# HKUST-KnowComp/DualMessagePassing

Hardware: AMD Instinct MI355X
Metric: (pattern,graph) pairs/sec DMPNN fwd+bwd hid=128 (higher is better)
Workload: dtype f32

## Files before the change

### dualmessagepassing_amd/_abi.py

```python
import ctypes

c_int = ctypes.c_int
c_i32 = ctypes.c_int32
c_i64 = ctypes.c_int64
c_u64 = ctypes.c_uint64
c_f32 = ctypes.c_float
c_double = ctypes.c_double
c_ptr = ctypes.c_void_p
c_size = ctypes.c_size_t

ABI_VERSION = 90

DMP_COLLATE_MAX_JOBS = 4
DMP_POOL_MAX_JOBS = 4
DMP_REDUCE_MAX_SEGMENTS = 16
DMP_ADAMW_MAX_SKIP = 16
DMP_ADAMW_MAX_SEGMENTS = 1024
DMP_LOOKUP_MAX_JOBS = 8
DMP_CONCAT_MAX_JOBS = 12
DMP_GEMM_MAX_JOBS = 12
DMP_GEMM_MAX_TERMS = 3
DMP_ATB_MAX_JOBS = 8
DMP_MEM_MEAN, DMP_MEM_SUM, DMP_MEM_MAX = 0, 1, 2


class dmp_collate_job(ctypes.Structure):
    _fields_ = [("local_src", c_ptr), ("local_dst", c_ptr), ("num_nodes", c_ptr), ("num_edges", c_ptr), ("B", c_i64), ("N", c_i64),
                ("E", c_i64), ("node_off", c_ptr), ("edge_off", c_ptr), ("src", c_ptr), ("dst", c_ptr), ("edge_graph", c_ptr),
                ("node_graph", c_ptr)]


class dmp_pool_job(ctypes.Structure):
    _fields_ = [("sizes_a", c_ptr), ("sizes_b", c_ptr), ("Ba", c_i64), ("Bb", c_i64), ("flag_a", c_ptr), ("flag_b", c_ptr),
                ("rows_a", c_i64), ("R", c_i64), ("chunk", c_int), ("off", c_ptr), ("gptr", c_ptr), ("vptr", c_ptr), ("vent", c_ptr),
                ("gent", c_ptr), ("seg", c_ptr), ("flag8", c_ptr), ("rowmap", c_ptr), ("sizes", c_ptr)]


class dmp_smallk_job(ctypes.Structure):
    _fields_ = [("X", c_ptr), ("ldx", c_i64), ("D", c_ptr), ("ldd", c_i64), ("gate", c_ptr), ("rowmask", c_ptr), ("R", c_i64),
                ("partial", c_ptr)]


class dmp_l0_pack_job(ctypes.Structure):
    _fields_ = [("enc_p", c_ptr), ("ldp", c_i64), ("rows_p", c_i64), ("enc_g", c_ptr), ("ldg", c_i64), ("gate", c_ptr), ("rows_g", c_i64),
# ... 233 lines not shown
    "dmp_atb_typed_blocks_h": (c_i64, [c_i64, c_int]),
    "dmp_atb_rows_blocks_h": (c_i64, [c_i64, c_int, c_int, c_int]),
    "dmp_atb_rows_plain": (c_int, [c_ptr, c_i64, c_ptr, c_i64, c_ptr, c_i64, c_int, c_int, c_int, c_ptr, c_ptr]),
    "dmp_atb_rows_masked": (c_int, [c_ptr, c_i64, c_ptr, c_i64, c_ptr, c_ptr, c_i64, c_int, c_int, c_int, c_ptr, c_ptr, c_ptr]),
    "dmp_atb_jobs_blocks_h": (c_i64, [c_i64, c_int, c_int]),
    "dmp_atb_rows_jobs_h": (c_int, [_p(dmp_atb_job), c_int, c_i64, c_int, c_ptr, c_ptr, c_ptr, c_i64, c_ptr]),
    "dmp_atb_tile_jobs_blocks": (c_i64, [c_i64, c_int, c_int]),
    "dmp_mfma_partial_rows_h": (c_i64, [c_i64, c_int]),
    "dmp_gemm_k64": (c_int, [c_ptr, c_i64, c_ptr, c_i64, c_int, c_ptr, c_i64, c_i64, c_ptr]),
    "dmp_atb_typed": (c_int, [c_ptr, c_i64, c_ptr, c_i64, c_ptr, c_ptr, c_ptr, c_i64, c_i64, c_int, c_ptr, c_ptr, c_ptr]),
    "dmp_out_fwd_fused_rows": (c_int, [c_ptr, c_i64, c_ptr, c_i64, c_ptr, c_ptr, c_ptr, c_int, c_ptr, c_i64, c_i64, c_int, c_int, c_ptr,
                                       c_i64, c_ptr]),
    "dmp_bwd_h1_fused_rows": (c_int, [c_ptr, c_i64, c_ptr, c_i64, c_ptr, c_i64, c_ptr, c_ptr, c_ptr, c_int, c_i64, c_int, c_f32, c_ptr,
                                      c_i64, c_ptr, c_ptr, c_ptr]),
    "dmp_kept_rows_scratch_words": (c_i64, [c_i64]),
    "dmp_kept_rows": (c_int, [c_ptr, c_i64, c_int, c_ptr, c_ptr, c_ptr, c_ptr]),
    "dmp_l0_edge_fwd_rows": (c_int, [c_ptr, c_i64, c_int, c_ptr, c_i64, c_ptr, c_i64, c_ptr, c_ptr, c_ptr, c_ptr, c_ptr, c_ptr, c_i64, c_int,
                                     c_f32, c_ptr, c_i64, c_ptr]),
    "dmp_l0_bwd_w_rows": (c_int, [c_ptr, c_i64, c_int, c_ptr, c_ptr, c_i64, c_ptr, c_i64, c_ptr, c_ptr, c_i64, c_int, c_ptr, c_ptr]),
    "dmp_typed_partial_rows": (c_i64, [c_i64, c_int]),
    "dmp_out_fwd_typed": (c_int, [_p(dmp_typed_job), c_int, c_ptr, c_ptr, c_ptr, c_i64, c_i64, c_int, c_ptr]),
    "dmp_bwd_h1_typed": (c_int, [c_ptr, c_i64, c_ptr, c_i64, c_ptr, c_i64, c_ptr, c_ptr, c_ptr, c_i64, c_i64, c_int, c_f32, c_ptr, c_i64,
                                 c_ptr, c_ptr, c_ptr]),
    "dmp_kept_rows_jobs": (c_int, [_p(dmp_kept_job), c_int, c_ptr, c_ptr, c_ptr, c_ptr, c_i64, c_ptr, c_ptr, c_ptr, c_ptr]),
    "dmp_row_mask_bits_jobs": (c_int, [_p(dmp_rowmask_job), c_int, c_ptr]),
    "dmp_atb2_blocks": (c_i64, [c_i64, c_int]),
    "dmp_atb2_jobs": (c_int, [_p(dmp_atb2_job), c_int, c_ptr, c_ptr, c_ptr, c_i64, c_i64, c_int, c_ptr]),
    "dmp_bwd_z_w": (c_int, [c_ptr, c_i64, c_ptr, c_i64, c_ptr, c_i64, c_ptr, c_i64, c_i64, c_ptr, c_i64, c_ptr, c_ptr, c_f32, c_f32,
                            c_ptr, c_ptr, c_ptr, c_i64, c_i64, c_int, c_ptr, c_i64, c_ptr, c_i64, c_ptr, c_ptr]),
    "dmp_out_fwd_typed_codes": (c_int, [_p(dmp_typed_job), c_ptr, c_i64, c_int, c_ptr, c_i64, c_i64, c_i64, c_ptr, c_ptr, c_ptr, c_i64, c_i64, c_int, c_ptr]),
    "dmp_bwd_h1_w_blocks": (c_i64, [c_i64]),
    "dmp_bwd_h1_w": (c_int, [c_ptr, c_i64, c_ptr, c_i64, c_ptr, c_i64, c_ptr, c_ptr, c_i64, c_i64, c_int, c_f32, c_ptr, c_i64,
                             c_ptr, c_ptr, c_ptr, c_ptr]),
    "dmp_row_mask_bits": (c_int, [c_ptr, c_i64, c_ptr, c_ptr]),
    "dmp_row_mask_rows": (c_int, [c_ptr, c_i64, c_int, c_i64, c_ptr, c_ptr]),
    "dmp_bwd_z_fused": (c_int, [c_ptr, c_i64, c_ptr, c_i64, c_ptr, c_i64, c_i64, c_ptr, c_i64, c_ptr, c_ptr, c_ptr,
                                c_f32, c_f32, c_i64, c_int, c_ptr, c_i64, c_ptr]),
    "dmp_gemm_k128": (c_int, [c_ptr, c_i64, c_ptr, c_i64, c_int, c_ptr, c_i64, c_i64, c_int, c_ptr]),
    "dmp_edge_combine": (c_int, [c_ptr, c_i64, c_ptr, c_i64, c_ptr, c_ptr, c_ptr, c_ptr, c_ptr, c_i64,
                                 c_int, c_int, c_f32, c_ptr, c_i64, c_ptr]),
    "dmp_relu_bwd_g_colsum": (c_int, [c_ptr, c_i64, c_ptr, c_i64, c_ptr, c_ptr, c_i64, c_int, c_f32, c_ptr, c_i64,
                                      c_ptr, c_ptr]),
    "dmp_edge_combine_bwd_g": (c_int, [c_ptr, c_i64, c_ptr, c_ptr, c_i64, c_int, c_ptr, c_i64, c_ptr]),
    "dmp_compgcn_agg": (c_int, [c_ptr, c_i64, c_ptr, c_i64, c_ptr, c_ptr, c_ptr, c_ptr, c_i64, c_int, c_int,
                                c_ptr, c_i64, c_ptr]),
    "dmp_compgcn_agg_bwd": (c_int, [c_ptr, c_i64, c_ptr, c_i64, c_ptr, c_i64, c_ptr, c_ptr, c_ptr, c_ptr,
                                    c_i64, c_int, c_int, c_ptr, c_i64, c_ptr, c_i64, c_ptr]),
    "dmp_attn_supported_dh": (c_int, [c_int]),
    "dmp_attn_fwd": (c_int, [c_ptr, c_ptr, c_ptr, c_ptr, c_ptr, c_i64, c_i64, c_i64, c_int, c_int, c_f32, c_ptr, c_ptr, c_ptr, c_ptr]),
    "dmp_attn_bwd": (c_int, [c_ptr, c_ptr, c_ptr, c_ptr, c_ptr, c_ptr, c_ptr, c_ptr, c_i64, c_i64, c_i64, c_int, c_int, c_f32, c_ptr,
                             c_ptr, c_ptr, c_ptr, c_ptr]),
    "dmp_mem_init_fwd": (c_int, [c_ptr, c_i64, c_ptr, c_i64, c_ptr, c_i64, c_i64, c_int, c_int, c_int, c_int, c_int, c_ptr, c_ptr,
                                 c_ptr, c_ptr, c_ptr, c_ptr, c_ptr]),
    "dmp_mem_init_bwd": (c_int, [c_ptr, c_ptr, c_ptr, c_ptr, c_ptr, c_i64, c_i64, c_int, c_int, c_int, c_int, c_ptr, c_ptr, c_ptr]),
    "dmp_cnn_fwd": (c_int, [c_ptr, c_i64, c_i64, c_int, c_ptr, c_ptr, c_int, c_int, c_int, c_int, c_int, c_f32, c_ptr, c_int, c_ptr,
                            c_ptr, c_ptr, c_ptr, c_ptr]),
    "dmp_cnn_route_bwd": (c_int, [c_ptr, c_ptr, c_ptr, c_i64, c_i64, c_i64, c_int, c_int, c_int, c_f32, c_ptr, c_ptr]),
    "dmp_cnn_wgrad_chunks": (c_i64, [c_i64]),
    "dmp_cnn_wgrad": (c_int, [c_ptr, c_ptr, c_i64, c_i64, c_i64, c_int, c_int, c_int, c_ptr, c_ptr]),
    "dmp_rnn_fwd": (c_int, [c_ptr, c_ptr, c_ptr, c_ptr, c_ptr, c_i64, c_i64, c_int, c_int, c_int, c_ptr, c_ptr, c_ptr, c_ptr]),
    "dmp_rnn_bwd": (c_int, [c_ptr, c_ptr, c_ptr, c_ptr, c_ptr, c_i64, c_i64, c_int, c_int, c_int, c_ptr, c_ptr]),
    "dmp_relconv_supported": (c_int, [c_int, c_int]),
    "dmp_relconv_fwd": (c_int, [c_ptr, c_ptr, c_ptr, c_ptr, c_ptr, c_ptr, c_ptr, c_i64, c_int, c_int, c_int, c_int, c_int, c_ptr,
                                c_ptr]),
    "dmp_relconv_bwd": (c_int, [c_ptr, c_ptr, c_ptr, c_ptr, c_ptr, c_ptr, c_ptr, c_i64, c_int, c_int, c_int, c_int, c_int, c_ptr,
                                c_ptr]),
# ... 2 lines not shown
```

### dualmessagepassing_amd/_build.py

```python
import fcntl
import hashlib
import os
import shutil
import subprocess
import tempfile

_HERE = os.path.dirname(os.path.abspath(__file__))
CSRC = os.path.join(_HERE, "csrc")
LIB_PATH = os.path.join(CSRC, "libdmp_hip.so")
HASH_PATH = LIB_PATH + ".srchash"
SOURCES = ["dmp_agg.hip", "dmp_segacc.hip", "dmp_compact.hip", "dmp_graph.hip", "dmp_fused.hip", "dmp_mfma.hip", "dmp_typed.hip", "dmp_h1w.hip", "dmp_atb.hip", "dmp_fold.hip", "dmp_heads.hip", "dmp_layer0.hip", "dmp_bn.hip", "dmp_attn.hip", "dmp_mem.hip", "dmp_cnn.hip", "dmp_rnn.hip", "dmp_relconv.hip",
           "dmp_subiso.cpp"]
HEADERS = ["dmp_common.h", "dmp_mfma_common.h", os.path.join("..", "..", "include", "dmp_hip.h")]
ARCH = "gfx950"
FLAGS = ["-O3", "-std=c++17", "-fPIC", "-ffp-contract=off", "-Wall", "-Wno-unused-function"]


def find_hipcc():
    for cand in (os.environ.get("HIPCC"), shutil.which("hipcc"), "/opt/rocm/bin/hipcc"):
        if cand and os.path.exists(cand):
            return cand
    return None


def source_hash():
    h = hashlib.sha256()
    h.update((ARCH + " ".join(FLAGS)).encode())
    for f in SOURCES + HEADERS:
        with open(os.path.join(CSRC, f), "rb") as fh:
            h.update(f.encode())
            h.update(fh.read())
    return h.hexdigest()


def _stale():
    if not os.path.exists(LIB_PATH) or not os.path.exists(HASH_PATH):
        return True
    with open(HASH_PATH) as f:
        return f.read().strip() != source_hash()


def build_lib(force=False, verbose=False):
    if not force and not _stale():
        return LIB_PATH
# ... 43 lines not shown
```

### dualmessagepassing_amd/fused.py

```python
import threading

import torch
from torch.autograd.function import once_differentiable

from . import _abi, _lib, ops
from ._lib import check, ptr, stream_ptr


def _partials(rows, H, dev):
    lib = _lib.load()
    return torch.empty((int(lib.dmp_colsum_partial_rows(rows, H)), H), dtype=torch.float32, device=dev)


MAX_REDUCE_SEGMENTS = _abi.DMP_REDUCE_MAX_SEGMENTS


class _Deferred(threading.local):

    def __init__(self):
        self.stack = []


_deferred = _Deferred()

# ... 617 lines not shown
USE_OUT_CODES = True


def out_codes_ok(h1, enc, K, Wc):
    lib = _lib.load()
    lim = (1 << 32) - 65536
    return bool(USE_OUT_CODES and h1.size(1) == 128 and not lib.dmp_dev_get_exact_fp32() and 1 <= K <= 16 and Wc.size(0) == K and Wc.size(1) == 128
                and enc.dtype == torch.float32 and enc.stride(1) == 1 and enc.stride(0) % 4 == 0 and enc.data_ptr() % 16 == 0
                and enc.size(0) == h1.size(0) and h1.size(0) * 128 * 4 < lim and Wc.stride(1) == 1)


def out_fwd_typed_codes(h1, W2t, b2, enc, K, Wc, tiles, prev=None, out=None, w_in_out=True, row0=0):
    lib = _lib.load()
    slot_edge, tile_scale, num_tiles, bound = tiles
    R, H = h1.shape
    if out is None:
        out = dead_rows_buffer((R, H), h1.device)
    Wc = Wc.detach()
    _lib.require_gpu(h1, W2t, out, prev, b2, enc, Wc)
    j = _abi.dmp_typed_job()
    j.Hin, j.ldh, j.W2, j.ldw, j.w_in_out = h1.data_ptr(), h1.stride(0), W2t.data_ptr(), W2t.stride(0), int(bool(w_in_out))
    j.bias = ptr(b2)
    j.R, j.ldr = ptr(prev), (prev.stride(0) if prev is not None else H)
    j.R2, j.ldr2 = None, H
    j.act, j.slope = 0, 0.0
    j.out, j.ldo = out.data_ptr(), out.stride(0)
    with _lib.timed("out_fwd_typed_codes[H=%d,R=%d]", (H, R), 4 * H * R * 2 + 4 * enc.size(1) * R):
        check(lib.dmp_out_fwd_typed_codes(_ctypes.byref(j), ptr(enc), enc.stride(0), int(K), ptr(Wc), Wc.stride(0), int(row0),
                                          0 if prev is None else min(R, prev.size(0)), ptr(slot_edge), ptr(tile_scale),
                                          ptr(num_tiles), bound, R, H, stream_ptr()), "dmp_out_fwd_typed_codes")
    return out


def out_fwd_typed(h1, W2t, b2, prev, tiles, out=None, w_in_out=True, slope=None, prev2=None):
    R, H = h1.shape
    if out is None:
        out = dead_rows_buffer((R, H), h1.device)
    typed_jobs([dict(a=h1, W=W2t, bias=b2, prev=prev, prev2=prev2, out=out, w_in_out=w_in_out, slope=slope)], tiles)
    return out


def bwd_h1_typed(d_o, W2, h1, tiles, slope=0.0, out=None):
    lib = _lib.load()
    E, H = d_o.shape
    slot_edge, tile_scale, num_tiles, bound = tiles
    d_g = out if out is not None else dead_rows_buffer((E, H), d_o.device)
    G = int(lib.dmp_typed_partial_rows(bound, H))
    part = torch.empty((G, H), dtype=torch.float32, device=d_o.device)
    part_rows = torch.empty_like(part)
    W2 = W2.contiguous()
    with _lib.timed("bwd_h1_typed[H=%d,E=%d]", (H, E), 12 * H * E + 4 * E):
        check(lib.dmp_bwd_h1_typed(ptr(d_o), d_o.stride(0), ptr(W2), W2.size(1), ptr(h1), h1.stride(0), ptr(slot_edge), ptr(tile_scale),
                                   ptr(num_tiles), bound, E, H, slope, ptr(d_g), d_g.stride(0), ptr(part), ptr(part_rows), stream_ptr()),
              "dmp_bwd_h1_typed")
    return d_g, reduce_partials(part), reduce_partials(part_rows)


def h1w_ok(d_o, h1, H):
    lib = _lib.load()
    return (H == 128 and not lib.dmp_dev_get_exact_fp32() and d_o.size(0) * d_o.stride(0) * 4 < (1 << 32) - 65536
            and h1.size(0) * h1.stride(0) * 4 < (1 << 32) - 65536 and d_o.size(0) * H * 4 < (1 << 32) - 65536)


def bwd_h1_w(d_o, W2, h1, tiles, slope=0.0, out=None):
    lib = _lib.load()
    E, H = d_o.shape
    slot_edge, _, num_tiles, bound = tiles
    d_g = out if out is not None else dead_rows_buffer((E, H), d_o.device)
    G = int(lib.dmp_bwd_h1_w_blocks(bound))
    part = torch.empty((G, H), dtype=torch.float32, device=d_o.device)
# ... 787 lines not shown
            XP = torch.empty((N, 3 * H), dtype=torch.float32, device=z.device)
            for t, (n0, n1) in l0.vtables(N):
                smallk_embed(l0.venc[n0:n1, :VK], MV[t * VK:(t + 1) * VK], None, XP[n0:n1], H)
        else:
            XP = x @ Wx
        if l0 is not None and node_pass:
            PXr, ldpx = PX, 2 * H
        else:
            PXr, ldpx = XP[:, H:], 3 * H
            if l0 is not None or nd is None:
                H1n = add_bias_relu_(SB, XP[:, :H], bn, slope)
        if nd is not None:
            xn = dead_rows_buffer((N, H), z.device) if (inner & 1) else torch.zeros((N, H), dtype=torch.float32, device=z.device)
            if nW2t is not None:
                out_fwd_typed(H1n, nW2t, nb2, x if residual else None, nd.tiles, out=xn)
            else:
                out_fwd_typed(H1n, nW2, nb2, x if residual else None, nd.tiles, out=xn, w_in_out=False)
        elif onepanel_ok(H):
            xn = out_fwd_mfma(H1n, nW2, nb2, v_gate, x if residual else None, nW2t)
        else:
            xn = gate_residual(x if residual else None, torch.addmm(nb2, H1n, nW2.t()), v_gate)
        sums_only = epool is not None and not edge_rows
        zn = None
        side.wait("erows" if l0 is not None else "tiles")
        dead_gate = e_gate if (SKIP_DEAD_ROWS and USE_ROW_MASKS and e_gate is not None and typed_ok(index, H)
                               and gate_row_mask(e_gate) is not None) else None
        if l0 is not None:
            H1e = dead_rows_buffer((z.size(0), H), z.device) if dead_gate is not None else torch.empty((z.size(0), H), dtype=torch.float32, device=z.device)
            for t, rows, _ in tables:
                if rows[1] > rows[0]:
                    l0_edge_fwd(enc0, K0, M0[t * K0:(t + 1) * K0], PXr, ldpx, be, coef, index, slope, rows, H1e,
                                mask=gate_row_mask(dead_gate) if dead_gate is not None else None)
        elif typed_ok(index, H):
            H1e = edge_fwd_typed(z, Wes, PXr, ldpx, be, coef, index, slope, dead_gate=dead_gate, sel=None if nd is None else nd.sel)
        elif mfma_ok(index, H):
            H1e = edge_fwd_mfma(z, Wes, PXr, ldpx, be, coef, index, slope)
        else:
            G = z @ Wes
            H1e = edge_combine_raw(G, 2 * H, PXr, ldpx, be, coef, index, H, relu=True, slope=slope)
            del G
            if not sums_only:
                Oe = torch.addmm(eb2, H1e, eW2.t())
                zn = gate_residual(z if residual else None, Oe, e_gate)
        if zn is None and not sums_only:
            dead = (3 if (inner & 1) else 1) if (dead_gate is not None and zero_rows_gate(e_gate)) else 0
            side.wait("tiles")
            lt = live_tiles(index, coef, e_gate) if (dead == 3 and eW2t is not None) else None
            if lt is not None:
                tl_ = ascending_tiles(e_gate) or lt
                if l0 is not None and residual and getattr(l0, "z_from_codes", False) and out_codes_ok(H1e, l0.enc, l0.K, W0[-l0.K:]):
                    zn = out_fwd_typed_codes(H1e, eW2t, eb2, l0.enc, l0.K, W0[-l0.K:], tl_, prev=l0.z_head, row0=l0.z_head.size(0))
                else:
                    zn = out_fwd_typed(H1e, eW2t, eb2, l0_rows(l0, W0, z) if residual else None, tl_)
            elif (l0 is not None and residual and e_gate is None and getattr(l0, "z_from_codes", False) and eW2t is not None
                  and out_codes_ok(H1e, l0.enc, l0.K, W0[-l0.K:]) and identity_tiles(H1e.size(0), H1e.device) is not None):
                zn = out_fwd_typed_codes(H1e, eW2t, eb2, l0.enc, l0.K, W0[-l0.K:], identity_tiles(H1e.size(0), H1e.device), prev=l0.z_head,
                                         row0=l0.z_head.size(0))
            else:
                zn = out_fwd_mfma(H1e, eW2, eb2, e_gate, l0_rows(l0, W0, z) if residual else None, eW2t, dead_rows=dead)
        ctx.index, ctx.coef, ctx.residual, ctx.H = index, coef, residual, H
        ctx.v_gate, ctx.e_gate, ctx.WesT, ctx.slope = v_gate, e_gate, WesT, slope
        ctx.vpool, ctx.epool = vpool, epool
        ctx.inner = int(inner)
        ctx.nd = nd
        ctx.l0, ctx.l0_S0, ctx.l0_tables = l0, S0, tables
        ctx.l0_W = None if l0 is None else (W0.detach(), None if WV0 is None else WV0.detach())
        ctx.save_for_backward(x, z if l0 is None else None, S, H1n, H1e, Bn, Wx, Wes, nW2, eW2)
# ... 315 lines not shown
```

### include/dmp_hip.h

```cpp
#ifndef DMP_HIP_H
#define DMP_HIP_H

#include <stddef.h>
#include <stdint.h>

#ifdef __cplusplus
extern "C" {
#endif

#define DMP_OK 0
#define DMP_ERR_BAD_ARG (-1)
#define DMP_ERR_UNSUPPORTED (-2)
#define DMP_ERR_HIP (-3)

#define DMP_ABI_VERSION 90
int dmp_abi_version(void);
const char *dmp_last_hip_error(void);


size_t dmp_csr_workspace_words(int64_t num_nodes, int64_t num_edges);

int dmp_csr_build(const int64_t *key, const uint8_t *flag, int64_t num_edges,
                  int64_t num_nodes, int32_t *rowptr, int32_t *ent,
                  int32_t *key32, int64_t *degree, int32_t *status,
                  int32_t *ws, void *stream);

size_t dmp_csr_pair_workspace_words(int64_t num_nodes);
int dmp_csr_build_pair(const int64_t *dst, const int64_t *src, const uint8_t *flag, int64_t num_edges, int64_t num_nodes,
                       int32_t *in_ptr, int32_t *in_ent, int32_t *dst32, int64_t *in_deg,
                       int32_t *out_ptr, int32_t *out_ent, int32_t *src32, int64_t *out_deg,
                       int32_t *status, int32_t *ws, void *stream);

int dmp_csr_build_graphs_max_nodes(void);
int dmp_csr_build_graphs(const int64_t *dst, const int64_t *src, const uint8_t *flag, const int64_t *node_off,
                         const int64_t *edge_off, int64_t B, int64_t E, int64_t N, int32_t *in_ptr, int32_t *in_ent,
                         int32_t *dst32, int64_t *in_deg, int32_t *out_ptr, int32_t *out_ent, int32_t *src32,
                         int64_t *out_deg, int32_t *status, void *stream);

int dmp_incidence_build(const int32_t *in_ptr, const int32_t *in_ent,
                        const int32_t *out_ptr, const int32_t *out_ent,
                        int64_t num_nodes, int64_t num_edges, int32_t *inc_ptr,
                        int32_t *inc_ent, void *stream);

int dmp_degree_coef(const int64_t *out_deg, int64_t num_nodes, float *coef,
                    void *stream);

int dmp_collate(const int64_t *local_src, const int64_t *local_dst,
                const int64_t *num_nodes, const int64_t *num_edges,
// ... 433 lines not shown
  const float *bias;
  const float *R; int64_t ldr;
  const float *R2; int64_t ldr2;
  int act; float slope;
  float *out; int64_t ldo;
} dmp_typed_job;
int dmp_out_fwd_typed(const dmp_typed_job *jobs, int num_jobs, const int32_t *slot_edge, const float *tile_scale,
                      const int32_t *num_tiles, int64_t tiles_bound, int64_t E, int H, void *stream);
int dmp_bwd_h1_typed(const float *dO, int64_t ldo, const float *W2, int64_t ldw, const float *H1, int64_t ldh,
                     const int32_t *slot_edge, const float *tile_scale, const int32_t *num_tiles, int64_t tiles_bound, int64_t E,
                     int H, float slope, float *dG, int64_t ldg, float *partial, float *partial_rows, void *stream);
int dmp_out_fwd_typed_codes(const dmp_typed_job *job, const float *codes, int64_t ldc, int kcodes, const float *Wc, int64_t ldwc,
                            int64_t code_row0, int64_t r_rows, const int32_t *slot_edge, const float *tile_scale, const int32_t *num_tiles, int64_t tiles_bound, int64_t E,
                            int H, void *stream);

typedef struct {
  const float *Z; int64_t ldz;
  const float *D; int64_t ldd;
  float *partial_T, *partial_B; int64_t partial_stride; int ldp;
} dmp_atb2_job;
int64_t dmp_atb2_blocks(int64_t tiles_bound, int num_jobs);
int dmp_atb2_jobs(const dmp_atb2_job *jobs, int num_jobs, const int32_t *slot_row, const float *tile_scale, const int32_t *num_tiles,
                  int64_t tiles_bound, int64_t rows, int H, void *stream);

int dmp_bwd_z_w(const float *dPre, int64_t ldp, const float *Z, int64_t ldz, const float *W, int64_t ldw, const float *D, int64_t ldd,
                int64_t num_nodes, const float *base, int64_t ldb, const int32_t *dst, const uint8_t *flag, float s0, float s1,
                const int32_t *slot_edge, const float *tile_scale, const int32_t *num_tiles, int64_t tiles_bound, int64_t E, int H,
                const int32_t *base_map, int64_t base_rows, float *dZ, int64_t ldo, float *partial_w, void *stream);
int64_t dmp_bwd_h1_w_blocks(int64_t tiles_bound);
int dmp_bwd_h1_w(const float *dO, int64_t ldo, const float *W2, int64_t ldw, const float *H1, int64_t ldh,
                 const int32_t *slot_edge, const int32_t *num_tiles, int64_t tiles_bound, int64_t E, int H, float slope,
                 float *dG, int64_t ldg, float *partial, float *partial_rows, float *partial_w, void *stream);

int dmp_bwd_z_fused(const float *dPre, int64_t ldp, const float *W, int64_t ldw,
                    const float *D, int64_t ldd, int64_t num_nodes, const float *base, int64_t ldb,
                    const float *coefE, const int32_t *dst, const uint8_t *flag, float s0,
                    float s1, int64_t num_edges, int H, float *dZ, int64_t ldz, void *stream);

int dmp_edge_fwd_typed(const float *Z, int64_t ldz, const float *W, int64_t ldw, const float *P,
                       int64_t ldp, int64_t num_nodes, const float *bias, const int32_t *selA,
                       const int32_t *selB, const int32_t *slot_edge, const float *tile_scale,
                       const int32_t *num_tiles, int64_t tiles_bound, int64_t num_edges, int H,
                       float slope, float *H1, int64_t ldh, void *stream);
int dmp_mask_slots(const int32_t *slot, int64_t n, const float *gate, int64_t E, int32_t *out, void *stream);
int dmp_bwd_z_typed_arow(const float *dPre, int64_t ldp, const float *W, int64_t ldw, const float *D, int64_t ldd,
                         int64_t num_nodes, const float *base, int64_t ldb, const int32_t *dst, const uint8_t *flag,
                         float s0, float s1, const int32_t *slot_edge, const int32_t *slot_arow, const float *tile_scale,
                         const int32_t *num_tiles, int64_t tiles_bound, int64_t E, int H, int w_transposed,
                         const int32_t *base_map, int64_t base_rows, float *dZ, int64_t ldz, void *stream);

int64_t dmp_atb_typed_blocks_h(int64_t tiles_bound, int H);
int dmp_atb_typed(const float *Z, int64_t ldz, const float *dPre, int64_t ldp,
                  const int32_t *slot_edge, const float *tile_scale, const int32_t *num_tiles,
                  int64_t tiles_bound, int64_t num_edges, int H, float *partial_T,
                  float *partial_B, void *stream);

int64_t dmp_atb_rows_blocks_h(int64_t rows, int M, int N, int H);
int dmp_atb_rows_masked(const float *A, int64_t lda, const float *B, int64_t ldb, const float *gate, const uint32_t *rowmask,
                        int64_t rows, int M, int N, int H, float *partial, float *partial_colsum, void *stream);
int dmp_atb_rows_plain(const float *A, int64_t lda, const float *B, int64_t ldb, const uint32_t *rowmask, int64_t rows, int M, int N,
                       int H, float *partial, void *stream);

int dmp_rel_gemm(const float *A, int64_t lda, int64_t rows_a, const float *W, int64_t ldw, int num_rels,
                 int w_transposed, const int32_t *slot_arow, const int32_t *slot_row,
                 const int32_t *tile_type, const int32_t *num_tiles, int64_t tiles_bound,
                 const float *row_scale, int64_t rows_c, int H, float *C, int64_t ldc, void *stream);
// ... 69 lines not shown
```

Measured before the change: 475,200.

## Fuse edge MLP first and second linear layers into one warp-specialized kernel

Adds a new HIP kernel that computes the first typed edge linear (with gather of node projections, bias and activation) and feeds its output through LDS directly into the second linear with bias and residual. Waves 0-3 produce H1 tiles and waves 4-7 consume them, using split-bf16 MFMA with a double-buffered LDS handoff. The aim is to avoid a separate launch and the global-memory round trip of H1 into the second GEMM. H1 is still written for backward. The cost is a complex producer/consumer schedule, one block per CU with large LDS, and a grid capped at 256 blocks.

```diff
diff --git a/dualmessagepassing_amd/_abi.py b/dualmessagepassing_amd/_abi.py
--- a/dualmessagepassing_amd/_abi.py
+++ b/dualmessagepassing_amd/_abi.py
@@ -9,7 +9,7 @@
 c_ptr = ctypes.c_void_p
 c_size = ctypes.c_size_t
 
-ABI_VERSION = 90
+ABI_VERSION = 91
 
 DMP_COLLATE_MAX_JOBS = 4
 DMP_POOL_MAX_JOBS = 4
@@ -309,6 +309,8 @@
     "dmp_bwd_h1_w_blocks": (c_i64, [c_i64]),
     "dmp_bwd_h1_w": (c_int, [c_ptr, c_i64, c_ptr, c_i64, c_ptr, c_i64, c_ptr, c_ptr, c_i64, c_i64, c_int, c_f32, c_ptr, c_i64,
                              c_ptr, c_ptr, c_ptr, c_ptr]),
+    "dmp_edge_mlp_fwd_typed": (c_int, [c_ptr, c_i64, c_ptr, c_i64, c_ptr, c_i64, c_i64, c_ptr, c_ptr, c_ptr, c_ptr, c_i64, c_ptr, c_int,
+                                       c_ptr, c_ptr, c_ptr, c_i64, c_i64, c_int, c_f32, c_ptr, c_i64, c_ptr, c_i64, c_ptr]),
     "dmp_row_mask_bits": (c_int, [c_ptr, c_i64, c_ptr, c_ptr]),
     "dmp_row_mask_rows": (c_int, [c_ptr, c_i64, c_int, c_i64, c_ptr, c_ptr]),
     "dmp_bwd_z_fused": (c_int, [c_ptr, c_i64, c_ptr, c_i64, c_ptr, c_i64, c_i64, c_ptr, c_i64, c_ptr, c_ptr, c_ptr,
diff --git a/dualmessagepassing_amd/_build.py b/dualmessagepassing_amd/_build.py
--- a/dualmessagepassing_amd/_build.py
+++ b/dualmessagepassing_amd/_build.py
@@ -9,7 +9,7 @@
 CSRC = os.path.join(_HERE, "csrc")
 LIB_PATH = os.path.join(CSRC, "libdmp_hip.so")
 HASH_PATH = LIB_PATH + ".srchash"
-SOURCES = ["dmp_agg.hip", "dmp_segacc.hip", "dmp_compact.hip", "dmp_graph.hip", "dmp_fused.hip", "dmp_mfma.hip", "dmp_typed.hip", "dmp_h1w.hip", "dmp_atb.hip", "dmp_fold.hip", "dmp_heads.hip", "dmp_layer0.hip", "dmp_bn.hip", "dmp_attn.hip", "dmp_mem.hip", "dmp_cnn.hip", "dmp_rnn.hip", "dmp_relconv.hip",
+SOURCES = ["dmp_agg.hip", "dmp_segacc.hip", "dmp_compact.hip", "dmp_graph.hip", "dmp_fused.hip", "dmp_mfma.hip", "dmp_typed.hip", "dmp_h1w.hip", "dmp_emlp.hip", "dmp_atb.hip", "dmp_fold.hip", "dmp_heads.hip", "dmp_layer0.hip", "dmp_bn.hip", "dmp_attn.hip", "dmp_mem.hip", "dmp_cnn.hip", "dmp_rnn.hip", "dmp_relconv.hip",
            "dmp_subiso.cpp"]
 HEADERS = ["dmp_common.h", "dmp_mfma_common.h", os.path.join("..", "..", "include", "dmp_hip.h")]
 ARCH = "gfx950"
diff --git a/dualmessagepassing_amd/csrc/dmp_emlp.hip b/dualmessagepassing_amd/csrc/dmp_emlp.hip
--- /dev/null
+++ b/dualmessagepassing_amd/csrc/dmp_emlp.hip
@@ -0,0 +1,372 @@
+#include "dmp_mfma_common.h"
+
+namespace dmp {
+namespace {
+
+struct EmlpArgs {
+  const float *Z; int64_t ldz;
+  const float *W; int64_t ldw;
+  const float *P; int64_t ldp; int64_t num_nodes;
+  const float *bias;
+  const int32_t *selA, *selB;
+  const float *W2; int64_t ldw2;
+  const float *bias2;
+  int residual;
+  float *H1; int64_t ldh;
+  float *Zn; int64_t ldo;
+  int64_t E;
+  const int32_t *slot_edge;
+  const float *tile_scale;
+  const int32_t *num_tiles;
+  float slope;
+};
+
+constexpr int kHE = 128, kThreadsE = 512;
+constexpr int kPlaneE = 32 * 256;
+constexpr int kBufE = 3 * kPlaneE;
+constexpr int kOpE = 2 * kBufE;
+constexpr int kImgE = 2 * kOpE;
+constexpr int kScrE = 8 * 32 * kScrStride * 4;
+constexpr int kRowE = 3 * kSub * 4;
+constexpr int kEmlpLdsBytes = kImgE + kScrE + kRowE;
+
+__device__ __forceinline__ uint32_t swz_e(uint32_t row) { return ((row & 3u) << 2) | ((row >> 2) & 3u); }
+
+__global__ __launch_bounds__(kThreadsE, 1) void emlp_fwd_k(const EmlpArgs p) {
+  extern __shared__ __attribute__((aligned(256))) unsigned char lds[];
+  uint32_t *const rowC = reinterpret_cast<uint32_t *>(lds + kImgE + kScrE);
+  const int wave = __builtin_amdgcn_readfirstlane((int)(threadIdx.x >> 6));
+  const bool second = wave >= 4;
+  const int lane = threadIdx.x & 63, li = lane & 31, h = lane >> 5;
+  constexpr uint32_t kNone = 0xFFFFFFFFu, kOOB = 0xFFFFF000u;
+
+  const int ntiles = __builtin_amdgcn_readfirstlane(*p.num_tiles);
+  const int chunk = (ntiles + (int)gridDim.x - 1) / (int)gridDim.x;
+  const int lo = (int)blockIdx.x * chunk;
+  const int hi = lo + chunk < ntiles ? lo + chunk : ntiles;
+  const int mine = hi > lo ? hi - lo : 0;
+  if (mine == 0) return;
+  const rsrc_t rs_slot = make_rsrc(p.slot_edge, (uint32_t)ntiles * (kSub * 4u));
+
+  const int cs = wave & 3;
+  const int col = 32 * cs + li;
+  float *const scr = reinterpret_cast<float *>(lds + kImgE) + wave * (32 * kScrStride);
+  const int lrow = lane >> 3, c4 = 32 * cs + (lane & 7) * 4;
+  const uint32_t col4 = (uint32_t)c4 * 4u;
+  constexpr int kGroups = 8;
+  Split8 B6[kGroups];
+  const uint32_t a0 = 256u * (uint32_t)li + 16u * ((uint32_t)(8 * h) ^ swz_e((uint32_t)li));
+  auto piece_off = [&](uint32_t r) { return 256u * r + 16u * ((uint32_t)(c4 >> 3) ^ swz_e(r)) + 8u * (uint32_t)((c4 >> 2) & 1); };
+  f32x16 acc;
+  auto product = [&](const unsigned char *img, auto &&action) {
+#pragma unroll
+    for (int r = 0; r < 16; ++r) acc[r] = 0.f;
+    Frag8 ah, am, al;
+    ah.v = *reinterpret_cast<const bf16x8 *>(img + a0);
+    am.v = *reinterpret_cast<const bf16x8 *>(img + kPlaneE + a0);
+    al.v = *reinterpret_cast<const bf16x8 *>(img + 2 * kPlaneE + a0);
+#pragma unroll
+    for (int g = 0; g < kGroups; ++g) {
+      Frag8 nh = ah, nm = am, nl = al;
+      if (g + 1 < kGroups) {
+        const uint32_t an = a0 ^ (uint32_t)(16 * (g + 1));
+        nh.v = *reinterpret_cast<const bf16x8 *>(img + an);
+        nm.v = *reinterpret_cast<const bf16x8 *>(img + kPlaneE + an);
+        nl.v = *reinterpret_cast<const bf16x8 *>(img + 2 * kPlaneE + an);
+      }
+      const Split8 &bb = B6[g];
+      __builtin_amdgcn_sched_barrier(0);
+      acc = __builtin_amdgcn_mfma_f32_32x32x16_bf16(al.v, bb.hi.v, acc, 0, 0, 0);
+      acc = __builtin_amdgcn_mfma_f32_32x32x16_bf16(ah.v, bb.lo.v, acc, 0, 0, 0);
+      acc = __builtin_amdgcn_mfma_f32_32x32x16_bf16(am.v, bb.mid.v, acc, 0, 0, 0);
+      __builtin_amdgcn_sched_barrier(0);
+      action(2 * g);
+      __builtin_amdgcn_sched_barrier(0);
+      acc = __builtin_amdgcn_mfma_f32_32x32x16_bf16(am.v, bb.hi.v, acc, 0, 0, 0);
+      acc = __builtin_amdgcn_mfma_f32_32x32x16_bf16(ah.v, bb.mid.v, acc, 0, 0, 0);
+      acc = __builtin_amdgcn_mfma_f32_32x32x16_bf16(ah.v, bb.hi.v, acc, 0, 0, 0);
+      __builtin_amdgcn_sched_barrier(0);
+      action(2 * g + 1);
+      ah = nh; am = nm; al = nl;
+    }
+  };
+  auto transpose_acc = [&]() {
+#pragma unroll
+    for (int r = 0; r < 16; ++r) scr[((r & 3) + 8 * (r >> 2) + 4 * h) * kScrStride + li] = acc[r];
+  };
+
+  if (second) {
+    const int u = threadIdx.x & 255;
+    const int srow = u >> 5, scol = u & 31;
+    const srsrc_t rs_Z = make_srsrc(p.Z, p.ldz, p.E);
+    const srsrc_t rs_O = make_srsrc(p.Zn, p.ldo, p.E);
+    const bool residual = __builtin_amdgcn_readfirstlane(p.residual) != 0;
+    float4 bias4 = make_float4(0.f, 0.f, 0.f, 0.f);
+    if (p.bias2) bias4 = *reinterpret_cast<const float4 *>(p.bias2 + c4);
+    int id_rows[kSubLoads];
+    int id_own = -1, own_staged = -1;
+    float4 pre[kSubLoads];
+    auto load_ids = [&](int k) {
+      const bool ok = k < mine;
+      const uint32_t so = (uint32_t)(lo + k) * (kSub * 4u);
+#pragma unroll
+      for (int m = 0; m < kSubLoads; ++m)
+        id_rows[m] = ok ? (int)__builtin_amdgcn_raw_buffer_load_b32(rs_slot, (srow + 8 * m) * 4, (int)so, 0) : -1;
+      if (u < kSub) id_own = ok ? (int)__builtin_amdgcn_raw_buffer_load_b32(rs_slot, u * 4, (int)so, 0) : -1;
+    };
+    auto load_row = [&](int m) { pre[m] = sbuf_load4(rs_Z, id_rows[m], (uint32_t)scol * 16u); };
+    auto stage_row = [&](int buf, int m) {
+      uint2 ph, pm, pl;
+      split_pair(pre[m].x, pre[m].y, ph.x, pm.x, pl.x);
+      split_pair(pre[m].z, pre[m].w, ph.y, pm.y, pl.y);
+      const uint32_t r = (uint32_t)(srow + 8 * m);
+      const uint32_t off = (uint32_t)buf * kBufE + 256u * r + 16u * ((uint32_t)(scol >> 1) ^ swz_e(r)) + 8u * (uint32_t)(scol & 1);
+      *reinterpret_cast<uint2 *>(lds + off) = ph;
+      *reinterpret_cast<uint2 *>(lds + off + kPlaneE) = pm;
+      *reinterpret_cast<uint2 *>(lds + off + 2 * kPlaneE) = pl;
+    };
+    auto stage_scalars = [&](int par) {
+      if (u < kSub) rowC[par * kSub + u] = own_staged >= 0 ? (uint32_t)own_staged : kNone;
+    };
+    auto load_panel = [&]() {
+      const rsrc_t rs_W = make_rsrc(p.W2, (uint32_t)(kHE * p.ldw2 * 4));
+      uint32_t off;
+      const uint32_t w_first = (uint32_t)((int64_t)64 * h * p.ldw2 + col) * 4u;
+      asm volatile("v_mov_b32 %0, %1" : "=v"(off) : "v"(w_first));
+      const uint32_t w_step = __builtin_amdgcn_readfirstlane((int)(p.ldw2 * 4));
+#pragma unroll
+      for (int s0 = 0; s0 < 64; s0 += 32) {
+        float w0[32];
+#pragma unroll
+        for (int j = 0; j < 32; ++j) w0[j] = __uint_as_float(__builtin_amdgcn_raw_buffer_load_b32(rs_W, (int)off, (int)((s0 + j) * w_step), 0));
+#pragma unroll
+        for (int q = 0; q < 32; q += 8)
+          split8(make_float4(w0[q], w0[q + 1], w0[q + 2], w0[q + 3]), make_float4(w0[q + 4], w0[q + 5], w0[q + 6], w0[q + 7]), B6[(s0 + q) / 8]);
+        __builtin_amdgcn_sched_barrier(0);
+      }
+    };
+    auto shadow = [&](int i, int k) {
+      if (i >= 4 && i < 8) stage_row((k + 1) & 1, i - 4);
+      else if (i == 8) stage_scalars((k + 1) % 3);
+      else if (i >= 9 && i < 13) load_row(i - 9);
+      else if (i == 13) { if (u < kSub) own_staged = id_own; }
+      else if (i == 14) load_ids(k + 3);
+    };
+    float4 res[4];
+#pragma unroll
+    for (int c = 0; c < 4; ++c) res[c] = make_float4(0.f, 0.f, 0.f, 0.f);
+    auto rebuild = [&](uint32_t hh, uint32_t mm, uint32_t ll, float &x0, float &x1) {
+      const float r0 = __uint_as_float(mm << 16) + __uint_as_float(ll << 16);
+      const float r1 = __uint_as_float(mm & 0xFFFF0000u) + __uint_as_float(ll & 0xFFFF0000u);
+      const float h0 = __uint_as_float(hh << 16), h1 = __uint_as_float(hh & 0xFFFF0000u);
+      x0 = r0 == 0.f ? h0 : h0 + r0;
+      x1 = r1 == 0.f ? h1 : h1 + r1;
+    };
+    auto read_residual = [&](int buf) {
+#pragma unroll
+      for (int c = 0; c < 4; ++c) {
+        const unsigned char *q = lds + (uint32_t)buf * kBufE + piece_off((uint32_t)(8 * c + lrow));
+        const uint2 ph = *reinterpret_cast<const uint2 *>(q);
+        const uint2 pm = *reinterpret_cast<const uint2 *>(q + kPlaneE);
+        const uint2 pl = *reinterpret_cast<const uint2 *>(q + 2 * kPlaneE);
+        rebuild(ph.x, pm.x, pl.x, res[c].x, res[c].y);
+        rebuild(ph.y, pm.y, pl.y, res[c].z, res[c].w);
+      }
+    };
+    auto epilogue = [&](int par) {
+      transpose_acc();
+#pragma unroll
+      for (int c = 0; c < 4; ++c) {
+        const int rr = 8 * c + lrow;
+        float4 v = *reinterpret_cast<const float4 *>(&scr[rr * kScrStride + (lane & 7) * 4]);
+        v.x = (v.x + bias4.x) + res[c].x; v.y = (v.y + bias4.y) + res[c].y;
+        v.z = (v.z + bias4.z) + res[c].z; v.w = (v.w + bias4.w) + res[c].w;
+        sbuf_store4(v, rs_O, (int)rowC[par * kSub + rr], col4);
+      }
+    };
+
+    load_ids(0);
+#pragma unroll
+    for (int m = 0; m < kSubLoads; ++m) load_row(m);
+    if (u < kSub) own_staged = id_own;
+    load_ids(1);
+    load_panel();
+#pragma unroll
+    for (int m = 0; m < kSubLoads; ++m) stage_row(0, m);
+    stage_scalars(0);
+#pragma unroll
+    for (int m = 0; m < kSubLoads; ++m) load_row(m);
+    if (u < kSub) own_staged = id_own;
+    load_ids(2);
+    lds_barrier();
+    for (int k = 0; k <= mine; ++k) {
+      if (k == 0) {
+#pragma unroll
+        for (int i = 0; i < 16; ++i) shadow(i, k);
+      } else {
+        product(lds + kOpE + (uint32_t)((k - 1) & 1) * kBufE, [&](int i) { shadow(i, k); });
+        epilogue((k - 1) % 3);
+      }
+      if (k == mine) break;
+      if (residual) read_residual(k & 1);
+      lds_barrier();
+    }
+    return;
+  }
+
+  constexpr uint32_t kRowBytes = kHE * 4u;
+  const srsrc_t rs_H = make_srsrc(p.H1, p.ldh, p.E);
+  const srsrc_t rs_T = make_srsrc(p.P, p.ldp, p.num_nodes);
+  const uint32_t rows4 = (uint32_t)(p.E * 4);
+  const rsrc_t rs_selA = make_rsrc(p.selA, rows4);
+  const rsrc_t rs_selB = make_rsrc(p.selB, rows4);
+  const float slope = __builtin_bit_cast(float, __builtin_amdgcn_readfirstlane(__builtin_bit_cast(int, p.slope)));
+  float4 bias4 = make_float4(0.f, 0.f, 0.f, 0.f);
+  if (p.bias) bias4 = *reinterpret_cast<const float4 *>(p.bias + c4);
+  const rsrc_t rs_W = make_rsrc(p.W, (uint32_t)(kHE * p.ldw * 4));
+  const uint32_t w_first = (uint32_t)((int64_t)64 * h * p.ldw + col) * 4u;
+  const uint32_t w_step = __builtin_amdgcn_readfirstlane((int)(p.ldw * 4));
+  auto load_panel = [&](float c) {
+    uint32_t off;
+    asm volatile("v_mov_b32 %0, %1" : "=v"(off) : "v"(w_first));
+#pragma unroll
+    for (int s0 = 0; s0 < 64; s0 += 8) {
+      float w0[8], w1[8];
+#pragma unroll
+      for (int j = 0; j < 8; ++j) {
+        w0[j] = __uint_as_float(__builtin_amdgcn_raw_buffer_load_b32(rs_W, (int)off, (int)((s0 + j) * w_step), 0));
+        w1[j] = __uint_as_float(__builtin_amdgcn_raw_buffer_load_b32(rs_W, (int)off + (int)kRowBytes, (int)((s0 + j) * w_step), 0));
+      }
+      float w[8];
+#pragma unroll
+      for (int j = 0; j < 8; ++j) w[j] = w0[j] + c * w1[j];
+      split8(make_float4(w[0], w[1], w[2], w[3]), make_float4(w[4], w[5], w[6], w[7]), B6[s0 / 8]);
+      __builtin_amdgcn_sched_barrier(0);
+    }
+  };
+  int e0 = -1, e1 = -1, e2 = -1, idn = -1;
+  uint32_t a1 = 0, b1 = 0, a2 = 0, b2 = 0;
+  auto load_id = [&](int k) {
+    return k < mine ? (int)__builtin_amdgcn_raw_buffer_load_b32(rs_slot, li * 4, (int)((uint32_t)(lo + k) * (kSub * 4u)), 0) : -1;
+  };
+  auto load_sel = [&](int e, uint32_t &a, uint32_t &b) {
+    const uint32_t eo = e >= 0 ? (uint32_t)e * 4u : kOOB;
+    a = __builtin_amdgcn_raw_buffer_load_b32(rs_selA, (int)eo, 0, 0);
+    b = __builtin_amdgcn_raw_buffer_load_b32(rs_selB, (int)eo, 0, 0);
+  };
+  float4 g0[4], g1[4];
+  auto fetch_operand = [&](int e, uint32_t a, uint32_t b, int c) {
+    const int rr = 8 * c + lrow;
+    const bool ok = __shfl(e, rr) >= 0;
+    const uint32_t ra = __shfl(a, rr), rb = __shfl(b, rr);
+    g0[c] = sbuf_load4(rs_T, ok ? (int)ra : -1, col4);
+    g1[c] = sbuf_load4(rs_T, ok ? (int)rb : -1, col4 + kRowBytes);
+  };
+  auto epilogue = [&](int buf) {
+    transpose_acc();
+#pragma unroll
+    for (int c = 0; c < 4; ++c) {
+      const int rr = 8 * c + lrow;
+      float4 v = *reinterpret_cast<const float4 *>(&scr[rr * kScrStride + (lane & 7) * 4]);
+      v.x = act_fwd((v.x + (g0[c].x - g1[c].x)) + bias4.x, slope);
+      v.y = act_fwd((v.y + (g0[c].y - g1[c].y)) + bias4.y, slope);
+      v.z = act_fwd((v.z + (g0[c].z - g1[c].z)) + bias4.z, slope);
+      v.w = act_fwd((v.w + (g0[c].w - g1[c].w)) + bias4.w, slope);
+      sbuf_store4(v, rs_H, __shfl(e0, rr), col4);
+      uint2 ph, pm, pl;
+      split_pair(v.x, v.y, ph.x, pm.x, pl.x);
+      split_pair(v.z, v.w, ph.y, pm.y, pl.y);
+      unsigned char *q = lds + kOpE + (uint32_t)buf * kBufE + piece_off((uint32_t)rr);
+      *reinterpret_cast<uint2 *>(q) = ph;
+      *reinterpret_cast<uint2 *>(q + kPlaneE) = pm;
+      *reinterpret_cast<uint2 *>(q + 2 * kPlaneE) = pl;
+      fetch_operand(e1, a1, b1, c);
+    }
+  };
+  float sv = 0.f;
+  e0 = load_id(0); e1 = load_id(1); e2 = load_id(2); idn = load_id(3);
+  {
+    uint32_t a0_ = 0, b0_ = 0;
+    load_sel(e0, a0_, b0_);
+    load_sel(e1, a1, b1);
+    load_sel(e2, a2, b2);
+#pragma unroll
+    for (int c = 0; c < 4; ++c) fetch_operand(e0, a0_, b0_, c);
+  }
+  lds_barrier();
+  float c_have = 0.f;
+  bool have_panel = false;
+  for (int k = 0; k < mine; ++k) {
+    if ((k & 63) == 0) sv = k + lane < mine ? p.tile_scale[lo + k + lane] : 0.f;
+    const float c = __shfl(sv, k & 63);
+    if (!have_panel || __float_as_uint(c) != __float_as_uint(c_have)) {
+      load_panel(c);
+      c_have = c;
+      have_panel = true;
+    }
+    int e3 = -1;
+    uint32_t a3 = 0, b3 = 0;
+    product(lds + (uint32_t)(k & 1) * kBufE, [&](int i) {
+      if (i == 0) load_sel(idn, a3, b3);
+      else if (i == 1) { e3 = idn; idn = load_id(k + 4); }
+    });
+    epilogue(k & 1);
+    e0 = e1;
+    e1 = e2; a1 = a2; b1 = b2;
+    e2 = e3; a2 = a3; b2 = b3;
+    lds_barrier();
+  }
+}
+
+inline unsigned emlp_blocks(int64_t tiles_bound) {
+  const int64_t cap = 256;
+  return (unsigned)(tiles_bound < cap ? (tiles_bound > 0 ? tiles_bound : 1) : cap);
+}
+
+constexpr int kMaxDevicesE = 64;
+inline bool emlp_lds_ready() {
+  static bool done[kMaxDevicesE] = {};
+  int dev = 0;
+  if (hipGetDevice(&dev) != hipSuccess || dev < 0 || dev >= kMaxDevicesE) dev = 0;
+  if (done[dev]) return true;
+  const hipError_t e = hipFuncSetAttribute(reinterpret_cast<const void *>(&emlp_fwd_k), hipFuncAttributeMaxDynamicSharedMemorySize, kEmlpLdsBytes);
+  if (e != hipSuccess) { set_last_hip_error(e); return false; }
+  done[dev] = true;
+  return true;
+}
+
+}
+}
+
+using namespace dmp;
+
+extern "C" {
+
+int dmp_edge_mlp_fwd_typed(const float *Z, int64_t ldz, const float *W, int64_t ldw, const float *P, int64_t ldp, int64_t num_nodes,
+                           const float *bias, const int32_t *selA, const int32_t *selB, const float *W2t, int64_t ldw2, const float *bias2,
+                           int residual, const int32_t *slot_edge, const float *tile_scale, const int32_t *num_tiles, int64_t tiles_bound,
+                           int64_t E, int H, float slope, float *H1, int64_t ldh, float *Zn, int64_t ldo, void *stream) {
+  if (H != 128 || g_exact_fp32) return DMP_ERR_UNSUPPORTED;
+  if (E < 0 || num_nodes < 0 || tiles_bound < 0) return DMP_ERR_BAD_ARG;
+  if (!slope_ok(slope)) return DMP_ERR_UNSUPPORTED;
+  if (E == 0) return DMP_OK;
+  if (!Z || !W || !P || !selA || !selB || !W2t || !slot_edge || !tile_scale || !num_tiles || !H1 || !Zn || ldz < H || ldw < 2 * H ||
+      ldp < 2 * H || ldw2 < H || ldh < H || ldo < H)
+    return DMP_ERR_BAD_ARG;
+  if (ldz % 4 || ldh % 4 || ldo % 4 || ldp % 4 || !aligned16(Z) || !aligned16(H1) || !aligned16(Zn) || !aligned16(P) ||
+      (bias && !aligned16(bias)) || (bias2 && !aligned16(bias2)))
+    return DMP_ERR_UNSUPPORTED;
+  if (!stride_ok(ldp) || !stride_ok(ldz) || !stride_ok(ldh) || !stride_ok(ldo) || E >= ((int64_t)1 << 30) || num_nodes >= ((int64_t)1 << 31) ||
+      tiles_bound * kSub * 4 >= ((int64_t)1 << 32) - 8192 || (int64_t)H * ldw * 4 >= ((int64_t)1 << 32) - 8192 ||
+      (int64_t)H * ldw2 * 4 >= ((int64_t)1 << 32) - 8192 || !fits4g(E, ldz) || !fits4g(E, ldh) || !fits4g(E, ldo) || !fits4g(num_nodes, ldp))
+    return DMP_ERR_UNSUPPORTED;
+  if (!emlp_lds_ready()) return DMP_ERR_HIP;
+  EmlpArgs a{};
+  a.Z = Z; a.ldz = ldz; a.W = W; a.ldw = ldw; a.P = P; a.ldp = ldp; a.num_nodes = num_nodes; a.bias = bias; a.selA = selA; a.selB = selB;
+  a.W2 = W2t; a.ldw2 = ldw2; a.bias2 = bias2; a.residual = residual ? 1 : 0; a.H1 = H1; a.ldh = ldh; a.Zn = Zn; a.ldo = ldo; a.E = E;
+  a.slot_edge = slot_edge; a.tile_scale = tile_scale; a.num_tiles = num_tiles; a.slope = slope;
+  emlp_fwd_k<<<emlp_blocks(tiles_bound), kThreadsE, kEmlpLdsBytes, (hipStream_t)stream>>>(a);
+  return check_launch();
+}
+
+}
diff --git a/dualmessagepassing_amd/fused.py b/dualmessagepassing_amd/fused.py
--- a/dualmessagepassing_amd/fused.py
+++ b/dualmessagepassing_amd/fused.py
@@ -673,10 +673,38 @@
     return out
 
 
-def out_fwd_typed(h1, W2t, b2, prev, tiles, out=None, w_in_out=True, slope=None, prev2=None):
+USE_EDGE_MLP_FWD = True
+
+
+def edge_mlp_fwd_ok(z, H, W2t):
+    lib = _lib.load()
+    return bool(USE_EDGE_MLP_FWD and H == 128 and W2t is not None and W2t.stride(1) == 1 and not lib.dmp_dev_get_exact_fp32()
+                and z.size(0) * H * 4 < (1 << 32) - 65536)
+
+
+def _edge_mlp_fwd(h1, W2t, b2, residual, tiles, out, first):
+    lib = _lib.load()
+    slot_edge, tile_scale, num_tiles, bound = tiles
+    z, Wes, P, bias = first["z"], first["Wes"].contiguous(), first["P"], first["bias"]
+    sel_a, sel_b = first["sel"]
+    R, H = h1.shape
+    _lib.require_gpu(h1, W2t, out, z, Wes, P, b2, bias, sel_a, sel_b)
+    with _lib.timed("out_fwd_typed[H=%d,R=%d,jobs=%d]", (H, R, 1), 4 * H * R * 3):
+        check(lib.dmp_edge_mlp_fwd_typed(ptr(z), z.stride(0), ptr(Wes), Wes.size(1), ptr(P), int(first["ldp"]), int(first["num_nodes"]),
+                                         ptr(bias), ptr(sel_a), ptr(sel_b), ptr(W2t), W2t.stride(0), ptr(b2), int(bool(residual)),
+                                         ptr(slot_edge), ptr(tile_scale), ptr(num_tiles), bound, R, H, float(first["slope"]),
+                                         ptr(h1), h1.stride(0), ptr(out), out.stride(0), stream_ptr()), "dmp_edge_mlp_fwd_typed")
+
+
+def out_fwd_typed(h1, W2t, b2, prev, tiles, out=None, w_in_out=True, slope=None, prev2=None, first=None):
     R, H = h1.shape
     if out is None:
         out = dead_rows_buffer((R, H), h1.device)
+    if first is not None:
+        if not (w_in_out and slope is None and prev2 is None and (prev is None or prev is first["z"])):
+            raise ValueError("out_fwd_typed(first=...): a plain second Linear whose residual is the first Linear's input")
+        _edge_mlp_fwd(h1, W2t, b2, prev is not None, tiles, out, first)
+        return out
     typed_jobs([dict(a=h1, W=W2t, bias=b2, prev=prev, prev2=prev2, out=out, w_in_out=w_in_out, slope=slope)], tiles)
     return out
 
@@ -1530,7 +1558,20 @@
                     l0_edge_fwd(enc0, K0, M0[t * K0:(t + 1) * K0], PXr, ldpx, be, coef, index, slope, rows, H1e,
                                 mask=gate_row_mask(dead_gate) if dead_gate is not None else None)
         elif typed_ok(index, H):
-            H1e = edge_fwd_typed(z, Wes, PXr, ldpx, be, coef, index, slope, dead_gate=dead_gate, sel=None if nd is None else nd.sel)
+            sel = None if nd is None else nd.sel
+            ft = None
+            if not sums_only and edge_mlp_fwd_ok(z, H, eW2t):
+                if e_gate is None:
+                    ft = index.class_tiles(coef)
+                elif dead_gate is not None and zero_rows_gate(e_gate) and (inner & 1):
+                    ft = live_tiles(index, coef, e_gate)
+            if ft is not None:
+                sel_a, sel_b = (sel[0], sel[1]) if sel is not None else index.edge_select(coef)[:2]
+                H1e = dead_rows_buffer((z.size(0), H), z.device)
+                zn = out_fwd_typed(H1e, eW2t, eb2, z if residual else None, ft,
+                                   first=dict(z=z, Wes=Wes, P=PXr, ldp=ldpx, num_nodes=index.num_nodes, bias=be, sel=(sel_a, sel_b), slope=slope))
+            else:
+                H1e = edge_fwd_typed(z, Wes, PXr, ldpx, be, coef, index, slope, dead_gate=dead_gate, sel=sel)
         elif mfma_ok(index, H):
             H1e = edge_fwd_mfma(z, Wes, PXr, ldpx, be, coef, index, slope)
         else:
diff --git a/include/dmp_hip.h b/include/dmp_hip.h
--- a/include/dmp_hip.h
+++ b/include/dmp_hip.h
@@ -13,7 +13,7 @@
 #define DMP_ERR_UNSUPPORTED (-2)
 #define DMP_ERR_HIP (-3)
 
-#define DMP_ABI_VERSION 90
+#define DMP_ABI_VERSION 91
 int dmp_abi_version(void);
 const char *dmp_last_hip_error(void);
 
@@ -513,6 +513,11 @@
                  const int32_t *slot_edge, const int32_t *num_tiles, int64_t tiles_bound, int64_t E, int H, float slope,
                  float *dG, int64_t ldg, float *partial, float *partial_rows, float *partial_w, void *stream);
 
+int dmp_edge_mlp_fwd_typed(const float *Z, int64_t ldz, const float *W, int64_t ldw, const float *P, int64_t ldp, int64_t num_nodes,
+                           const float *bias, const int32_t *selA, const int32_t *selB, const float *W2t, int64_t ldw2, const float *bias2,
+                           int residual, const int32_t *slot_edge, const float *tile_scale, const int32_t *num_tiles, int64_t tiles_bound,
+                           int64_t num_edges, int H, float slope, float *H1, int64_t ldh, float *Zn, int64_t ldo, void *stream);
+
 int dmp_bwd_z_fused(const float *dPre, int64_t ldp, const float *W, int64_t ldw,
                     const float *D, int64_t ldd, int64_t num_nodes, const float *base, int64_t ldb,
                     const float *coefE, const int32_t *dst, const uint8_t *flag, float s0,
```

After: 476,600, median of 3. No clear change (+0.3%).
